# marius311/MuseInference.jl

Measured on AMD Instinct MI355X. Metric: MC sims/sec (MAP+score), higher is better.
Workload: dtype f64; 1 GPU; funnel_1e4: Neal's funnel family model=funnel, N=10000-dim z, 1-dim theta, nsims=512 per step (512 on this rank), cold start z0=0, atol=1e-2; element_split=1, parallelism=sims sharded over 1 GPU(s) (weak scaling), one all-gather of scores per step

## Files before the change

museinference.jl_amd/csrc/solver.hpp:

```cpp
#pragma once
#include <math.h>

#include "models.hpp"
#include "reduce.hpp"
#include "rng.hpp"

namespace muse {

template <int EPT>
struct Prefetch {
    int p;
    bool have_n1;
    bool have_n2;
    bool have_x;
    bool have_xg;
    bool g_pending;
};
#ifndef MUSE_NORMALS_AUX
#define MUSE_NORMALS_AUX 0
#endif
constexpr int kNormalsAux = MUSE_NORMALS_AUX;
typedef __attribute__((address_space(1))) const void* glds_src_t;
typedef __attribute__((address_space(3))) void* glds_dst_t;
template <int T, int EPT>
// ... 656 lines not shown
                dphi = trial_dphi;
                last_c = c;
                last_gmax = trial_gmax;
                last_phi = phi;
                f_calls += 1;
                return;
            }
        }
        double gm;
        if constexpr (!Place::kResident && !Model::kStencil) {
            if (z_zero) eval<true, false, false, true, kSpec>(c, phi, dphi, gm);
            else eval<true, false>(c, phi, dphi, gm);
        } else if constexpr (kSpec) {
            eval<true, false, false, false, true>(c, phi, dphi, gm);
        } else {
            eval<true, false>(c, phi, dphi, gm);
        }
        last_c = c;
        last_gmax = gm;
        last_phi = phi;
    }

    __device__ __forceinline__ static bool finite2(double p, double d) { return isfinite(p) && isfinite(d); }
    __device__ __forceinline__ static double eps_of(double b) {
        const double ab = fabs(b);
        return __longlong_as_double(__double_as_longlong(ab) + 1) - ab;
    }
    __device__ __forceinline__ static double nextup(double v) {
        if (v == 0.0) return 4.9406564584124654e-324;
        const long long b = __double_as_longlong(v);
        return __longlong_as_double(v > 0.0 ? b + 1 : b - 1);
    }
    __device__ __forceinline__ static bool wolfe(double c, double phi_c, double dphi_c, double phi_0, double dphi_0,
                                                 double phi_lim) {
        double delta = kHzDelta, sigma = kHzSigma, delta2 = 2.0 * kHzDelta - 1.0;
        if constexpr (Place::kResident) asm volatile("" : "+v"(delta), "+v"(sigma), "+v"(delta2));
        const bool w1 = (delta * dphi_0 >= (phi_c - phi_0) / c) && (dphi_c >= sigma * dphi_0);
        const bool w2 = (delta2 * dphi_0 >= dphi_c) && (dphi_c >= sigma * dphi_0) && (phi_c <= phi_lim);
        return w1 || w2;
    }
    __device__ __forceinline__ static double secant(const HzPoint& p, const HzPoint& q) {
        return (p.a * q.d - q.a * p.d) / (q.d - p.d);
    }

    __device__ __forceinline__ bool linesearch(double c0, double phi_0, double dphi_0, double& alpha) {
        enum { S_INIT, S_EXPAND, S_BIS, S_SEC1, S_SEC2, S_MID, S_FINAL };
        enum { CONT_BRACKET, CONT_UPD1, CONT_UPD2, CONT_UPD3 };
        alpha = 0.0;
        if (!finite2(phi_0, dphi_0)) return false;
        if (dphi_0 >= kEps * fabs(phi_0)) return false;
        if (dphi_0 >= 0.0 || c0 <= kEps) return true;
        const double phi_lim = phi_0 + kHzEpsilon * fabs(phi_0);
        const HzPoint P0{0.0, phi_0, dphi_0, 0};
        HzPoint A = P0, B = P0, C = P0, prev = P0, a0 = P0, b0 = P0;
        double alphamax = INFINITY, cold = 0.0, fail_alpha = 0.0, c = c0;
        int state = S_INIT, cont = CONT_BRACKET, iter = 1, iterfinite = 1, nid = 1;
        bool ok = true;
        for (;;) {
            double phi, dphi;
            if (iter_stamp < 3) stamp(stamp_p, 10 + 2 * iter_stamp);
            phidphi(c, phi, dphi);
            if (iter_stamp < 3) stamp(stamp_p, 11 + 2 * iter_stamp);
            iter_stamp += 1;
            const bool fin = finite2(phi, dphi);
            switch (state) {
                case S_INIT:
                    if (!fin) {
                        if (iterfinite < kHzIterFiniteMax) { iterfinite += 1; c *= kHzPsi3; continue; }
                        alpha = 0.0;
                        goto L_DONE;
                    }
                    C = HzPoint{c, phi, dphi, nid++};
                    goto L_BRACKET_TOP;
                case S_EXPAND:
                    if (!fin) {
                        if (c > nextup(cold) && iterfinite < kHzIterFiniteMax) {
                            alphamax = c;
                            iterfinite += 1;
                            c = (cold + c) / 2.0;
                            continue;
                        }
                        alpha = cold;
                        goto L_DONE;
                    }
                    C = HzPoint{c, phi, dphi, nid++};
                    iter += 1;
                    goto L_BRACKET_TOP;
                case S_BIS: {
                    if (!fin) goto L_FAIL;
                    const HzPoint D{c, phi, dphi, nid++};
                    if (D.d >= 0.0) { B = D; goto L_BISECT_RETURN; }
                    if (D.v <= phi_lim) A = D;
                    else B = D;
                    goto L_BISECT_TOP;
                }
                case S_SEC1:
                    if (!fin) goto L_FAIL;
                    C = HzPoint{c, phi, dphi, nid++};
                    if (wolfe(c, phi, dphi, phi_0, dphi_0, phi_lim)) { alpha = c; goto L_DONE; }
                    cont = CONT_UPD1;
                    goto L_UPDATE;
                case S_SEC2:
                    if (!fin) goto L_FAIL;
                    C = HzPoint{c, phi, dphi, nid++};
                    if (wolfe(c, phi, dphi, phi_0, dphi_0, phi_lim)) { alpha = c; goto L_DONE; }
                    cont = CONT_UPD2;
                    goto L_UPDATE;
                case S_MID:
                    if (!fin) goto L_FAIL;
                    C = HzPoint{c, phi, dphi, nid++};
                    cont = CONT_UPD3;
                    goto L_UPDATE;
                default:
                    return ok;
            }
        L_BRACKET_TOP:
            if (!(iter < kHzLinesearchMax)) { alpha = 0.0; goto L_FAIL_KEEP; }
            if (C.d >= 0.0) {
                A = prev;
                B = C;
                iter += 1;
                goto L_MAIN_TOP;
            } else if (C.v > phi_lim) {
                A = P0;
                B = C;
                cont = CONT_BRACKET;
                fail_alpha = 0.0;
                goto L_BISECT_ENTER;
            } else {
                cold = C.a;
                if (nextup(cold) >= alphamax) { alpha = cold; goto L_DONE; }
                prev = C;
                c = cold * kHzRho;
                if (c > alphamax) c = alphamax;
                iterfinite = 1;
                state = S_EXPAND;
                continue;
            }
        L_UPDATE:
            if (!(A.d < 0.0 && A.v <= phi_lim && B.d >= 0.0 && B.a > A.a)) goto L_FAIL;
            if (C.a < A.a || C.a > B.a) goto L_UPDATE_RETURN;
            if (C.d >= 0.0) { B = C; goto L_UPDATE_RETURN; }
            if (C.v <= phi_lim) { A = C; goto L_UPDATE_RETURN; }
            B = C;
        L_BISECT_ENTER:
            if (!(A.d < 0.0 && A.v <= phi_lim && B.d < 0.0 && B.v > phi_lim && B.a > A.a)) goto L_FAIL;
        L_BISECT_TOP:
            if (B.a - A.a > eps_of(B.a)) {
                c = (A.a + B.a) / 2.0;
                state = S_BIS;
                continue;
            }
        L_BISECT_RETURN:
            if (cont == CONT_BRACKET) { iter += 1; goto L_MAIN_TOP; }
        L_UPDATE_RETURN:
            if (cont == CONT_UPD1) {
                const bool updB = (B.id == C.id), updA = (A.id == C.id);
                double c2 = C.a;
                if (updB) c2 = secant(b0, B);
                else if (updA) c2 = secant(a0, A);
                if ((updA || updB) && A.a <= c2 && c2 <= B.a) {
                    c = c2;
                    state = S_SEC2;
                    continue;
                }
            }
            if (cont == CONT_UPD3) { iter += 1; goto L_MAIN_TOP; }
            if (!(B.a > A.a)) { alpha = A.a; goto L_FAIL_KEEP; }
            if (B.a - A.a < kHzGamma * (b0.a - a0.a)) {
                if (nextup(a0.v) >= b0.v && nextup(A.v) >= B.v) { alpha = A.a; goto L_DONE; }
                iter += 1;
                goto L_MAIN_TOP;
            }
            fail_alpha = A.a;
            c = (A.a + B.a) / 2.0;
            state = S_MID;
            continue;
        L_MAIN_TOP:
            if (!(iter < kHzLinesearchMax)) { alpha = A.a; goto L_FAIL_KEEP; }
            a0 = A;
            b0 = B;
            if (!(b0.a > a0.a)) { alpha = a0.a; goto L_FAIL_KEEP; }
            if (b0.a - a0.a <= eps_of(b0.a)) { alpha = a0.a; goto L_DONE; }
            fail_alpha = a0.a;
            if (!(a0.d < 0.0 && b0.d >= 0.0)) goto L_FAIL;
            c = secant(a0, b0);
            if (!isfinite(c)) goto L_FAIL;
            state = S_SEC1;
            continue;
        L_FAIL:
            alpha = fail_alpha;
        L_FAIL_KEEP:
            ok = false;
        L_DONE:
            if (!ok) return false;
            if (alpha == last_c) return true;
            c = alpha;
            state = S_FINAL;
        }
    }

    ProblemDesc d;
    double f, gmax;
    int iterations, hist_words, status;
    double* extra;

    __device__ __forceinline__ void run(int p, double* wg_scratch, double* lds_x, double* lds_g) {
        Prefetch<EPT> none;
        none.p = -1;
        none.g_pending = false;
        run(p, wg_scratch, lds_x, lds_g, none);
    }
    template <bool FD = true>
    __device__ __forceinline__ void run(int p, double* wg_scratch, double* lds_x, double* lds_g, Prefetch<EPT>& pf, int next_p = -1) {
        begin<false, FD>(p, wg_scratch, lds_x, lds_g, pf);
        if (d.normals_only) return;
        pfp = &pf;
        if constexpr (Place::kResident && Place::kXgLds) {
            if (next_p >= 0 && a.ncache_mode == 2 && !(a.debug & 4)) prefetch_issue<T>(a, tid, next_p, lds_x, lds_g, pf, false);
        }
        solve(p);
        finish(p);
        if constexpr (FD) {
            if (is_fid(p)) publish_fiducial();
        }
    }
    __device__ __forceinline__ bool is_fid(int p) const { return a.kind == BATCH_FD && a.fd_fold && p == 0; }
    __device__ __forceinline__ bool wait_fid(int p) const { return a.kind == BATCH_FD && a.fd_fold && p != 0; }
    __device__ __forceinline__ int info_row(int p) const {
        return (a.kind == BATCH_FD && a.fd_fold) ? (p == 0 ? a.nproblems - 1 : p - 1) : p;
    }
    __device__ __forceinline__ void publish_fiducial() {
        asm volatile("s_waitcnt vmcnt(0)" ::: "memory");
        __syncthreads();
        if (tid == 0) __hip_atomic_store(a.fid_flag, a.fid_tag, __ATOMIC_RELEASE, __HIP_MEMORY_SCOPE_AGENT);
    }
    __device__ __forceinline__ void wait_fiducial() {
        int* seen = reinterpret_cast<int*>(sh_rho + 40) + 2;
        if ((unsigned)__builtin_amdgcn_readfirstlane(seen[0]) == a.fid_tag) return;
        if ((__builtin_amdgcn_readfirstlane(tid) >> 6) == 0) {
            unsigned long long t0 = 0;
            unsigned spins = 0;
            while (__hip_atomic_load(a.fid_flag, __ATOMIC_RELAXED, __HIP_MEMORY_SCOPE_AGENT) != a.fid_tag) {
                __builtin_amdgcn_s_sleep(32);
                if ((++spins & 0x3fu) == 0) {
                    unsigned long long now;
                    asm volatile("s_memrealtime %0\n\ts_waitcnt lgkmcnt(0)" : "=s"(now)::"memory");
                    if (t0 == 0) t0 = now;
                    else if (now - t0 > 200000000ull) {
                        typedef __attribute__((address_space(1))) int gi32;
                        __hip_atomic_store((gi32*)a.error_flag, 1, __ATOMIC_RELAXED, __HIP_MEMORY_SCOPE_SYSTEM);
                        break;
                    }
                }
            }
        }
        __syncthreads();
        __builtin_amdgcn_fence(__ATOMIC_ACQUIRE, "agent");
        if (tid == 0) seen[0] = (int)a.fid_tag;
    }
#ifndef MUSE_KEEPZ_MAXB
#define MUSE_KEEPZ_MAXB 8
#endif
    static constexpr bool kKeepZ = Place::kResident && Place::kXgLds && !Model::kStencil && MAXB <= MUSE_KEEPZ_MAXB;
    __device__ __forceinline__ bool can_keep(int p) const {
        if constexpr (!kKeepZ) return false;
        const ProblemDesc dd = describe(a, p);
        return dd.z0_mode == Z0_WARM && !dd.normals_only && dd.tsample < 0 &&
               ((dd.x_mode == X_SAMPLE && dd.nslot >= 0 && a.ncache_mode == 2) || dd.x_mode == X_DATA);
    }
    __device__ __forceinline__ bool keeps_next(int p) const {
        if constexpr (!kKeepZ) return false;
        const ProblemDesc dd = describe(a, p);
        return !dd.normals_only && dd.tsample < 0 && dd.zslot >= 0 &&
               ((dd.x_mode == X_SAMPLE && dd.nslot >= 0 && a.ncache != nullptr && a.ncache_mode != 0) || dd.x_mode == X_DATA);
    }
    __device__ __forceinline__ void store_kept(int p) {
        if constexpr (kKeepZ) {
            const ProblemDesc dd = describe(a, p);
            if (dd.zslot < 0) return;
            const int64_t ld = a.ld;
            VH zout;
            zout.bind(a.zhat + dd.zslot * ld, ld);
            for_elems<T, EPT, U>(ld, tfirst, ps(), [&](int jj, int i) { zout.set(jj, i, z.get(jj, i)); });
        }
    }
    __device__ __forceinline__ void after_begin(int p, double* lds_x, double* lds_g, Prefetch<EPT>& pf, int next_p) {
        if (d.normals_only) return;
        pfp = &pf;
        if constexpr (Place::kResident && Place::kXgLds) {
            if (next_p >= 0 && a.ncache_mode == 2 && !(a.debug & 4)) prefetch_issue<T>(a, tid, next_p, lds_x, lds_g, pf, false);
        }
        solve(p);
        finish(p);
    }
    __device__ __forceinline__ void begin_kept(int p, double* wg_scratch, double* lds_x, double* lds_g, Prefetch<EPT>& pf) {
        if constexpr (kKeepZ) {
            d = describe(a, p);
            const bool pf_hit = pf.p == p;
            const int64_t N = a.N, ld = a.ld;
            init_done = false;
            z_zero = false;
            have_trial = false;
            stamp(p, 0);
            iv0 = a.cur.t.iv[0];
            sd0 = a.cur.t.sd[0];
            if constexpr (Model::kPair && MAXB == 2) {
                this->pc[0] = this->psd[0] = a.cur.t.sd[0];
                this->pc[1] = this->psd[1] = a.cur.t.sd[1];
                this->pc[2] = a.cur.t.sd[2];
                this->pc[3] = a.cur.t.sd[3];
            }
            if constexpr (MAXB > 1) {
                int tl = tid;
                asm volatile("" : "+v"(tl));
                if constexpr (Model::kPair) {
                    if (tl < MAXB) sh_sd[tl] = pair_table(a.cur.t)[4 * (tl >> 1) + (tl & 1)];
                } else {
                if (tl < MAXB) sh_sd[tl] = a.cur.t.sd[tl];
                }
                wg_barrier<true>();
            }
            hist = wg_scratch;
            x.bind(lds_x, ld);
            g.bind(lds_g, ld);
            if (d.x_mode == X_SAMPLE) {
                const rsrc_t n1r = make_rsrc(a.ncache + (int64_t)(2 * d.nslot) * ld, ld * 8);
                const rsrc_t n2r = make_rsrc(a.ncache + (int64_t)(2 * d.nslot + 1) * ld, ld * 8);
                int tl = tid;
                asm volatile("" : "+v"(tl));
                const bool n1_here = pf_hit && pf.have_n1, n2_here = pf_hit && pf.have_n2;
                if (n1_here && n2_here) {
                    asm volatile("s_waitcnt vmcnt(0)" ::: "memory");
#pragma unroll
                    for (int j = 0; j < EPT; ++j) {
                        const int i0 = 2 * (tl + j * T);
                        const double a0 = g.get(2 * j, i0), a1 = g.get(2 * j + 1, i0 + 1);
                        const double b0 = x.get(2 * j, i0), b1 = x.get(2 * j + 1, i0 + 1);
                        double zt0, xt0, zt1, xt1;
                        Model::sample(scoef(2 * j, i0), a0, b0, zt0, xt0, i0);
                        Model::sample(scoef(2 * j + 1, i0 + 1), a1, b1, zt1, xt1, i0 + 1);
                        const bool valid1 = i0 + 1 < (int)N;
                        if constexpr (Model::kPair) xt0 = i0 < (int)N ? xt0 : 0.0;
                        x.set(2 * j, i0, xt0);
                        x.set(2 * j + 1, i0 + 1, valid1 ? xt1 : 0.0);
                    }
                } else {
                    double c1[EPT][2], c2[EPT][2];
                    if (n1_here) asm volatile("s_waitcnt vmcnt(0)" ::: "memory");
                    if (!n2_here) {
#pragma unroll
                        for (int j = 0; j < EPT; ++j) load_f64x2<kNormalsAux>(n2r, 2 * (tl + j * T), c2[j][0], c2[j][1]);
                    }
                    if (!n1_here) {
#pragma unroll
                        for (int j = 0; j < EPT; ++j) load_f64x2<kNormalsAux>(n1r, 2 * (tl + j * T), c1[j][0], c1[j][1]);
                    }
                    if (n1_here) {
#pragma unroll
                        for (int j = 0; j < EPT; ++j) {
                            const int i0 = 2 * (tl + j * T);
                            c1[j][0] = g.get(2 * j, i0); c1[j][1] = g.get(2 * j + 1, i0 + 1);
                        }
                    }
                    if (n2_here) {
#pragma unroll
                        for (int j = 0; j < EPT; ++j) {
                            const int i0 = 2 * (tl + j * T);
                            c2[j][0] = x.get(2 * j, i0); c2[j][1] = x.get(2 * j + 1, i0 + 1);
                        }
                    }
#pragma unroll
                    for (int j = 0; j < EPT; ++j) {
                        const int i0 = 2 * (tl + j * T);
                        double zt0, xt0, zt1, xt1;
                        Model::sample(scoef(2 * j, i0), c1[j][0], c2[j][0], zt0, xt0, i0);
                        Model::sample(scoef(2 * j + 1, i0 + 1), c1[j][1], c2[j][1], zt1, xt1, i0 + 1);
                        const bool valid1 = i0 + 1 < (int)N;
                        if constexpr (Model::kPair) xt0 = i0 < (int)N ? xt0 : 0.0;
                        x.set(2 * j, i0, xt0);
                        x.set(2 * j + 1, i0 + 1, valid1 ? xt1 : 0.0);
                    }
                }
            } else {
                if (pf_hit && pf.have_x) {
                    asm volatile("s_waitcnt vmcnt(0)" ::: "memory");
                } else {
                    VH xs;
                    xs.bind(a.x_data, ld);
                    for_elems<T, EPT, U>(ld, tfirst, ps(), [&](int jj, int i) { x.set(jj, i, xs.get(jj, i)); }, x);
                }
            }
            s.clear();
            if (pf_hit) {
                pf.p = -1;
                pf.g_pending = false;
            }
            stamp(p, 9);
            wg_barrier<true>();
            stamp(p, 1);
        }
    }
    Prefetch<EPT>* pfp;
    __device__ __forceinline__ void drop_g_prefetch() {
        if constexpr (Place::kResident && Place::kXgLds) {
            if (pfp->g_pending) {
                asm volatile("s_waitcnt vmcnt(0)" ::: "memory");
                pfp->g_pending = false;
                pfp->p = -1;
            }
        }
    }

    __device__ __forceinline__ const SampleSd* tsample_base() const {
        if (a.tsample) return a.tsample;
        return reinterpret_cast<const SampleSd*>(reinterpret_cast<const char*>((const void*)__builtin_amdgcn_kernarg_segment_ptr()) +
                                                 offsetof(BatchArgs, maps));
    }
    template <bool KEEP_ZTRUE>
    __device__ __forceinline__ void begin(int p, double* wg_scratch, double* lds_x, double* lds_g) {
        Prefetch<EPT> none;
        none.p = -1;
        none.g_pending = false;
        pfp = nullptr;
        begin<KEEP_ZTRUE>(p, wg_scratch, lds_x, lds_g, none);
    }
    template <bool KEEP_ZTRUE, bool FD = true>
    __device__ __forceinline__ void begin(int p, double* wg_scratch, double* lds_x, double* lds_g, Prefetch<EPT>& pf) {
        d = describe(a, p);
        const bool pf_hit = Place::kResident && Place::kXgLds && pf.p == p;
        const int64_t N = a.N, ld = a.ld;
        init_done = false;
        z_zero = false;
        have_trial = false;
        stamp(p, 0);
        iv0 = a.cur.t.iv[0];
        sd0 = d.tsample >= 0 ? tsample_base()[d.tsample].sd[0] : a.cur.t.sd[0];
        if constexpr (Model::kPair && MAXB == 2) {
            this->pc[0] = a.cur.t.sd[0];
            this->pc[1] = a.cur.t.sd[1];
            this->pc[2] = a.cur.t.sd[2];
            this->pc[3] = a.cur.t.sd[3];
            this->psd[0] = sd0;
            this->psd[1] = d.tsample >= 0 ? tsample_base()[d.tsample].sd[1] : a.cur.t.sd[1];
        }
        if constexpr (kBig) {
            const BigTheta* bt = reinterpret_cast<const BigTheta*>(
                reinterpret_cast<const char*>((const void*)__builtin_amdgcn_kernarg_segment_ptr()) + offsetof(BatchArgs, big));
            big_iv = bt->iv;
            big_sd = d.tsample >= 0 ? reinterpret_cast<const double*>(a.tsample) + (int64_t)d.tsample * kBigTheta : bt->sd;
            big_rcpN = 1.0 / (double)a.N;
        } else if constexpr (MAXB > 1) {
            int tl = tid;
            asm volatile("" : "+v"(tl));
            if constexpr (Model::kPair) {
                if (tl < MAXB) sh_sd[tl] = d.tsample >= 0 ? tsample_base()[d.tsample].sd[tl] : pair_table(a.cur.t)[4 * (tl >> 1) + (tl & 1)];
            } else {
            if (tl < MAXB) sh_sd[tl] = d.tsample >= 0 ? tsample_base()[d.tsample].sd[tl] : a.cur.t.sd[tl];
            }
            wg_barrier<!Model::kStencil>();
        }
        const double* zmem = nullptr;
        if constexpr (Place::kResident) {
            hist = wg_scratch;
            if constexpr (Place::kXgLds) {
                x.bind(lds_x, ld);
                g.bind(lds_g, ld);
            }
        } else {
            double* xbuf = wg_scratch;
            double* sbuf = wg_scratch + 2 * ld;
            if constexpr (kBg) {
                if (bufsel) {
                    xbuf = wg_scratch + (int64_t)(4 + 2 * kM + 1) * ld;
                    sbuf = xbuf + ld;
                }
            }
            x.bind(xbuf, ld);
            g.bind(wg_scratch + ld, ld);
            if constexpr (Place::kLdsS) s.bind(wg_scratch + 2 * ld, ld, lds_x, tfirst, pstride, tid, (int)N);
            else s.bind(sbuf, ld);
            zmem = d.zslot >= 0 ? a.zhat + d.zslot * ld : wg_scratch + 3 * ld;
            z.bind(zmem, ld);
            hist = wg_scratch + 4 * ld;
            extra = hist + (int64_t)2 * kM * ld;
        }
        const double* z0ptr = a.zhat + d.z0slot * ld;
        VH z0src;
        z0src.bind(z0ptr, ld);
        const bool z_in_place = (!Place::kResident) && (d.z0_mode == Z0_WARM || d.z0_mode == Z0_COPY) && (z0ptr == zmem);

        if (d.x_mode == X_SAMPLE) {
            const uint64_t sim = (uint64_t)d.sim;
            if constexpr (Place::kResident && Place::kXgLds) {
                const int nmode = d.nslot >= 0 ? a.ncache_mode : 0;
                rsrc_t n1r = make_rsrc(a.ncache, 0), n2r = n1r;
                if (nmode != 0) {
                    n1r = make_rsrc(a.ncache + (int64_t)(2 * d.nslot) * ld, ld * 8);
                    n2r = make_rsrc(a.ncache + (int64_t)(2 * d.nslot + 1) * ld, ld * 8);
                }
                const bool z_warm = d.z0_mode != Z0_ZERO && d.z0_mode != Z0_TRUE;
                bool z_loaded = false;
                double zw[EPT][2];
                if (nmode == 2) {
                    double c1[EPT][2], c2[EPT][2];
                    int tl = tid;
                    asm volatile("" : "+v"(tl));
                    const bool n1_here = pf_hit && pf.have_n1, n2_here = pf_hit && pf.have_n2;
                    if (n1_here) asm volatile("s_waitcnt vmcnt(0)" ::: "memory");
                    const bool fold_wait = FD && wait_fid(p);
                    if (z_warm && !fold_wait) {
#pragma unroll
                        for (int j = 0; j < EPT; ++j) load_f64x2(z0src.rsrc, 2 * (tl + j * T), zw[j][0], zw[j][1]);
                        z_loaded = true;
                    }
                    if (!n2_here) {
#pragma unroll
                        for (int j = 0; j < EPT; ++j) load_f64x2<kNormalsAux>(n2r, 2 * (tl + j * T), c2[j][0], c2[j][1]);
                    }
                    if (!n1_here) {
#pragma unroll
                        for (int j = 0; j < EPT; ++j) load_f64x2<kNormalsAux>(n1r, 2 * (tl + j * T), c1[j][0], c1[j][1]);
                    }
                    if (n1_here) {
#pragma unroll
                        for (int j = 0; j < EPT; ++j) {
                            const int i0 = 2 * (tl + j * T);
                            c1[j][0] = g.get(2 * j, i0); c1[j][1] = g.get(2 * j + 1, i0 + 1);
                        }
                    }
                    if (n2_here) {
#pragma unroll
                        for (int j = 0; j < EPT; ++j) {
                            const int i0 = 2 * (tl + j * T);
                            c2[j][0] = x.get(2 * j, i0); c2[j][1] = x.get(2 * j + 1, i0 + 1);
                        }
                    }
                    const bool stage_ztrue = d.z0_mode == Z0_TRUE;
#pragma unroll
                    for (int j = 0; j < EPT; ++j) {
                        const int i0 = 2 * (tl + j * T);
                        double zt0, xt0, zt1, xt1;
                        Model::sample(scoef(2 * j, i0), c1[j][0], c2[j][0], zt0, xt0, i0);
                        Model::sample(scoef(2 * j + 1, i0 + 1), c1[j][1], c2[j][1], zt1, xt1, i0 + 1);
                        const bool valid1 = i0 + 1 < (int)N;
                        if constexpr (Model::kPair) {
                            const bool valid0 = i0 < (int)N;
                            xt0 = valid0 ? xt0 : 0.0;
                            zt0 = valid0 ? zt0 : 0.0;
                        }
                        x.set(2 * j, i0, xt0);
                        x.set(2 * j + 1, i0 + 1, valid1 ? xt1 : 0.0);
                        if (stage_ztrue) {
                            g.set(2 * j, i0, zt0);
                            g.set(2 * j + 1, i0 + 1, valid1 ? zt1 : 0.0);
                        }
                    }
                    if (z_warm && fold_wait) {
                        wait_fiducial();
#pragma unroll
                        for (int j = 0; j < EPT; ++j) load_f64x2(z0src.rsrc, 2 * (tl + j * T), zw[j][0], zw[j][1]);
                        z_loaded = true;
                    }
                } else {
                    auto sd_of = [&](int jj) {
                        if constexpr (MAXB == 1) return sd0;
                        else {
                            const unsigned w = jj >= 10 ? pk[1] : pk[0];
                            const int sh = 3 * (jj >= 10 ? jj - 10 : jj);
                            if constexpr (Model::kPair) return scoef_of_block((int)((w >> sh) & 7u));
                            else return sh_sd[(w >> sh) & 7u];
                        }
                    };
                    auto draw = [&](auto npairs, int i0, int j) {
                        constexpr int P = decltype(npairs)::value;
                        uint64_t idx[2 * P];
                        NormalPair np[2 * P];
#pragma unroll
                        for (int q = 0; q < P; ++q) {
                            idx[2 * q] = (uint64_t)(i0 + 2 * T * q);
                            idx[2 * q + 1] = (uint64_t)(i0 + 2 * T * q + 1);
                        }
                        normal_pairs<2 * P>(a.seed, sim, idx, np);
#pragma unroll
                        for (int q = 0; q < P; ++q) {
                            const int j0 = i0 + 2 * T * q;
                            if (nmode == 1) {
                                store_f64x2(n1r, j0, np[2 * q].n1, np[2 * q + 1].n1);
                                store_f64x2(n2r, j0, np[2 * q].n2, np[2 * q + 1].n2);
                            }
                            double zt0, xt0, zt1, xt1;
                            Model::sample(sd_of(2 * (j + q)), np[2 * q].n1, np[2 * q].n2, zt0, xt0, j0);
                            Model::sample(sd_of(2 * (j + q) + 1), np[2 * q + 1].n1, np[2 * q + 1].n2, zt1, xt1, j0 + 1);
                            const bool valid1 = j0 + 1 < (int)N;
                            x.p[j0] = xt0;
                            g.p[j0] = zt0;
                            x.p[j0 + 1] = valid1 ? xt1 : 0.0;
                            g.p[j0 + 1] = valid1 ? zt1 : 0.0;
                        }
                    };
                    int j = 0;
                    int tl = tid;
                    asm volatile("" : "+v"(tl));
#pragma unroll 1
                    for (int i0 = 2 * tl; i0 < (int)N; i0 += 2 * T * kSamplerPairs, j += kSamplerPairs) {
                        if constexpr (kSamplerPairs == 2) {
                            if (i0 + 2 * T < (int)N) draw(std::integral_constant<int, 2>{}, i0, j);
                            else draw(std::integral_constant<int, 1>{}, i0, j);
                        } else {
                            draw(std::integral_constant<int, 1>{}, i0, j);
                        }
                    }
                }
                z.clear();
                s.clear();
                if (z_loaded) {
#pragma unroll
                    for (int j = 0; j < EPT; ++j) {
                        z.set(2 * j, 0, zw[j][0]);
                        z.set(2 * j + 1, 0, zw[j][1]);
                    }
                } else {
                    for_elems<T, EPT, U>(ld, tfirst, ps(), [&](int jj, int i) {
                        if (d.z0_mode == Z0_ZERO) z.set(jj, i, 0.0);
                        else if (d.z0_mode == Z0_TRUE) z.set(jj, i, g.get(jj, i));
                        else z.set(jj, i, z0src.get(jj, i));
                    });
                }
            } else {
                x.clear(); g.clear(); z.clear(); s.clear();
                VH ztrue;
                if constexpr (KEEP_ZTRUE) ztrue.bind(extra, ld);
                constexpr int US = Place::kResident ? U : 1;
                const bool z_from_sample = d.z0_mode == Z0_ZERO || d.z0_mode == Z0_TRUE;
                if constexpr (kBg && !KEEP_ZTRUE) {
                    if (d.z0_mode == Z0_ZERO && !d.normals_only && d.tsample < 0) {
                        if (gen.p != p) {
                            gen.p = p;
                            gen.trip = 0;
                            gen.sim = sim;
#pragma unroll
                            for (int k = 0; k < 4; ++k) gen.sum[k] = 0.0;
                            gen.mx[0] = gen.mx[1] = 0.0;
                        }
                        gen.active = false;
                        const int ntrips = gen_trips();
#pragma unroll 1
                        for (; gen.trip < ntrips; ++gen.trip) {
                            const int i0 = 2 * (tfirst + gen.trip * pstride);
                            double xo[2], so[2];
                            gen_pair(i0, xo, so);
                            store_f64x2(x.rsrc, i0, xo[0], xo[1]);
                            store_f64x2(s.rsrc, i0, so[0], so[1]);
                        }
                        double sum[4] = {gen.sum[0], gen.sum[1], gen.sum[2], gen.sum[3]}, mx[2] = {gen.mx[0], gen.mx[1]};
                        reduce<4, 2>(sum, mx);
                        init_f = 0.5 * (sum[0] + a.cur.f_const);
                        init_dphi = sum[1];
                        init_gmax = nan_if(sum[0] != sum[0] || sum[1] != sum[1], mx[0]);
                        trial_c = 1.0;
                        trial_phi = 0.5 * (sum[2] + a.cur.f_const);
                        trial_dphi = sum[3];
                        trial_gmax = nan_if(sum[2] != sum[2] || sum[3] != sum[3], mx[1]);
                        init_done = true;
                        z_zero = true;
                    }
                }
                if constexpr (!Model::kStencil) {
                    if (!init_done && z_from_sample && !d.normals_only) {
                        const bool ztrue_start = d.z0_mode == Z0_TRUE;
                        double sum[4] = {0.0, 0.0, 0.0, 0.0}, mx[2] = {0.0, 0.0};
                        constexpr int kGenU = Place::kResident ? 1 : kStreamGenU;
                        NormalPair npv[2 * kGenU];
                        for_elems_pre<T, EPT, kGenU>(ld, tfirst, ps(), [&](auto ucount, int i0, int pstr) {
                            constexpr int UU = decltype(ucount)::value;
                            uint64_t idx[2 * UU];
                            NormalPair got[2 * UU];
#pragma unroll
                            for (int u = 0; u < UU; ++u) {
                                idx[2 * u] = (uint64_t)(i0 + 2 * u * pstr);
                                idx[2 * u + 1] = (uint64_t)(i0 + 2 * u * pstr + 1);
                            }
                            normal_pairs<2 * UU>(a.seed, sim, idx, got);
#pragma unroll
                            for (int q = 0; q < 2 * UU; ++q) npv[q] = got[q];
                        }, [&](int jj, int i) {
                            const bool valid = i < N;
                            const NormalPair np = npv[jj % (2 * kGenU)];
                            double zt, xt;
                            Model::sample(scoef(jj, i), np.n1, np.n2, zt, xt, i);
                            zt = valid ? zt : 0.0;
                            xt = valid ? xt : 0.0;
                            if constexpr (KEEP_ZTRUE) ztrue.set(jj, i, keep_value(valid, zt, sdk(jj, i), np, i));
                            x.set(jj, i, xt);
                            const double z0v = ztrue_start ? zt : 0.0;
                            if (Place::kResident || ztrue_start) z.set(jj, i, z0v);
                            const auto ivi = gcoef(jj, i);
                            const double gi = Model::grad(ivi, xt, z0v, sum[0], i);
                            const double sd = -gi;
                            s.set(jj, i, sd);
                            sum[1] = fma(gi, sd, sum[1]);
                            mx[0] = absmax(mx[0], gi);
                            const double zt1 = fma(1.0, sd, z0v);
                            const double gt = Model::grad(ivi, xt, zt1, sum[2], i);
                            sum[3] = fma(gt, sd, sum[3]);
                            mx[1] = absmax(mx[1], gt);
                        }, when(KEEP_ZTRUE, ztrue), x, s, when(Place::kResident || ztrue_start, z));
                        reduce<4, 2>(sum, mx);
                        init_f = 0.5 * (sum[0] + a.cur.f_const);
                        init_dphi = sum[1];
                        init_gmax = nan_if(sum[0] != sum[0] || sum[1] != sum[1], mx[0]);
                        trial_c = 1.0;
                        trial_phi = 0.5 * (sum[2] + a.cur.f_const);
                        trial_dphi = sum[3];
                        trial_gmax = nan_if(sum[2] != sum[2] || sum[3] != sum[3], mx[1]);
                        init_done = true;
                        z_zero = !ztrue_start && !Place::kResident;
                    }
                }
                if (!init_done)
                for_elems<T, EPT, US>(ld, tfirst, ps(), [&](int jj, int i) {
                    const bool valid = i < N;
                    const NormalPair np = normal_pair(a.seed, sim, (uint64_t)i);
                    double zt, xt;
                    if constexpr (Model::kStencil) {
                        zt = sdk(jj, i) * np.n1;
                        xt = np.n2;
                        g.set(jj, i, valid ? zt : 0.0);
                    } else {
                        Model::sample(scoef(jj, i), np.n1, np.n2, zt, xt, i);
                    }
                    zt = valid ? zt : 0.0;
                    xt = valid ? xt : 0.0;
                    if constexpr (KEEP_ZTRUE) ztrue.set(jj, i, keep_value(valid, zt, sdk(jj, i), np, i));
                    x.set(jj, i, xt);
                    if (d.z0_mode == Z0_ZERO) z.set(jj, i, 0.0);
                    else if (d.z0_mode == Z0_TRUE) z.set(jj, i, zt);
                    else if constexpr (Place::kResident) z.set(jj, i, z0src.get(jj, i));
                }, when(Model::kStencil, g), when(KEEP_ZTRUE, ztrue), x, when(z_from_sample, z));
                if constexpr (!Place::kResident) {
                    if (!init_done && !z_from_sample && !z_in_place)
                        for_elems<T, EPT, U>(ld, tfirst, ps(), [&](int jj, int i) { z.set(jj, i, z0src.get(jj, i)); }, z);
                }
            }
            if constexpr (Model::kStencil) {
                pass_barrier();
                const NoiseVec<Model, 1> sn;
                for_elems<T, EPT, U>(ld, tfirst, ps(), [&](int jj, int i) {
                    const bool valid = i < N;
                    const int ic = valid ? i : 0;
                    const int im = ic == 0 ? (int)N - 1 : ic - 1, ip = ic == (int)N - 1 ? 0 : ic + 1;
                    const double zl = g.get1(im), zr = g.get1(ip);
                    const double az = stencil_apply<Model>(zl, g.get1(ic), zr);
                    if constexpr (noise_model<Model>()) {
                        const double si = sn.get(jj, i);
                        const double xv = fma(si, x.get(jj, i), az);
                        x.set(jj, i, valid && si != 0.0 ? xv : 0.0);
                    } else {
                        const double xv = az + x.get(jj, i);
                        x.set(jj, i, valid ? xv : 0.0);
                    }
                }, x);
            }
        } else {
            VH xs;
            xs.bind(d.x_mode == X_DATA ? a.x_data : a.x_given, ld);
            x.clear(); g.clear(); z.clear(); s.clear();
            const bool z_zero = d.z0_mode == Z0_ZERO || d.z0_mode == Z0_TRUE;
            bool done = false;
            if constexpr (Place::kResident && Place::kXgLds) {
                if (pf_hit && pf.have_x && d.x_mode == X_DATA && !z_zero) {
                    asm volatile("s_waitcnt vmcnt(0)" ::: "memory");
                    for_elems<T, EPT, U>(ld, tfirst, ps(), [&](int jj, int i) { z.set(jj, i, z0src.get(jj, i)); });
                    done = true;
                } else if (pf_hit && pf.have_xg && d.x_mode == X_DATA && !z_zero) {
                    asm volatile("s_waitcnt vmcnt(0)" ::: "memory");
                    for_elems<T, EPT, U>(ld, tfirst, ps(), [&](int jj, int i) {
                        x.set(jj, i, g.get(jj, i));
                        z.set(jj, i, z0src.get(jj, i));
                    });
                    done = true;
                }
            }
            if (!done)
            for_elems<T, EPT, U>(ld, tfirst, ps(), [&](int jj, int i) {
                x.set(jj, i, xs.get(jj, i));
                if (z_zero) z.set(jj, i, 0.0);
                else if (!z_in_place) z.set(jj, i, z0src.get(jj, i));
            }, x, when(z_zero || !z_in_place, z));
        }
        if (pf_hit) {
            if constexpr (Place::kResident && Place::kXgLds) {
                if (pf.g_pending) asm volatile("s_waitcnt vmcnt(0)" ::: "memory");
            }
            pf.p = -1;
            pf.g_pending = false;
        }
        stamp(p, 9);
        if constexpr (Model::kStencil) pass_barrier();
        else wg_barrier<true>();
        if constexpr (kBg && !KEEP_ZTRUE) {
            gen.active = false;
            const bool same_map = a.nmaps <= 1 || next_p / a.n_per_map == p / a.n_per_map;
            if (next_p >= 0 && d.tsample < 0 && same_map) {
                const ProblemDesc dn = describe(a, next_p);
                if (dn.x_mode == X_SAMPLE && dn.z0_mode == Z0_ZERO && !dn.normals_only && dn.tsample < 0) {
                    gen.p = next_p;
                    gen.trip = 0;
                    gen.sim = (uint64_t)dn.sim;
#pragma unroll
                    for (int k = 0; k < 4; ++k) gen.sum[k] = 0.0;
                    gen.mx[0] = gen.mx[1] = 0.0;
                    gen.active = true;
                    double* xb = bufsel ? wg_scratch : wg_scratch + (int64_t)(4 + 2 * kM + 1) * ld;
                    double* sb = bufsel ? wg_scratch + 2 * ld : xb + ld;
                    bg_xr = make_rsrc(xb, ld * 8);
                    bg_sr = make_rsrc(sb, ld * 8);
                }
            }
        }

        stamp(p, 1);
    }

    static constexpr bool kPrefetchTwoLoop = !Place::kResident && Place::kCluster && Model::kStencil;
    template <class F>
    __device__ __forceinline__ void pass_ab(VH& A, VH& B, F&& f) {
        int t = tfirst;
        asm volatile("" : "+v"(t));
        const int n = (int)a.ld, pstr = pstride;
#pragma unroll 1
        for (int i0 = 2 * t; i0 < n; i0 += 2 * U * pstr) {
#pragma unroll
            for (int u = 0; u < U; ++u) {
                const int i = i0 + 2 * u * pstr;
                f(2 * u, i);
                f(2 * u + 1, i + 1);
            }
            s.template flush<U>(i0, pstr);
            A.unload();
            B.unload();
        }
    }
    __device__ __forceinline__ double twoloop_prefetched(int upper, int lower, double dot0) {
        if constexpr (kPrefetchTwoLoop) {
            double dot = dot0;
            int t0 = tfirst;
            asm volatile("" : "+v"(t0));
            auto fetch = [&](VH& v) { v.template preload<U>(2 * t0, pstride); };
            VH A = hdg((upper - 1) % kM), B = A;
            if (upper > lower) B = hdx((upper - 2) % kM);
            for (int index = upper; index >= lower; --index) {
                const int slot = (index - 1) % kM;
                const double al = sh_rho[slot] * dot;
                if ((tid & 63) == 0) sh_alpha[slot] = al;
                double sum[1] = {0.0}, mx[1] = {0.0};
                if (index > lower) {
                    pass_ab(A, B, [&](int jj, int i) {
                        const double qi = fma(-al, A.get(jj, i), s.get(jj, i));
                        s.set(jj, i, qi);
                        sum[0] = fma(B.get(jj, i), qi, sum[0]);
                    });
                } else {
                    const double gam = sh_gam[(upper - 1) % kM];
                    pass_ab(A, B, [&](int jj, int i) {
                        const double dgi = A.get(jj, i);
                        const double si = gam * fma(-al, dgi, s.get(jj, i));
                        s.set(jj, i, si);
                        sum[0] = fma(dgi, si, sum[0]);
                    });
                }
                if (index > lower) {
                    A = hdg((index - 2) % kM);
                    fetch(A);
                    if (index - 1 > lower) {
                        B = hdx((index - 3) % kM);
                        fetch(B);
                    }
                } else {
                    A = hdx((lower - 1) % kM);
                    fetch(A);
                    if (lower < upper) {
                        B = hdg(lower % kM);
                        fetch(B);
                    } else {
                        fetch(g);
                    }
                }
                reduce<1, 0>(sum, mx);
                dot = sum[0];
            }
            for (int index = lower; index <= upper; ++index) {
                const int slot = (index - 1) % kM;
                const double beta = sh_rho[slot] * dot;
                const double coef = sh_alpha[slot] - beta;
                double sum[1] = {0.0}, mx[1] = {0.0};
                if (index < upper) {
                    pass_ab(A, B, [&](int jj, int i) {
                        const double si = fma(A.get(jj, i), coef, s.get(jj, i));
                        s.set(jj, i, si);
                        sum[0] = fma(B.get(jj, i), si, sum[0]);
                    });
                    A = hdx(index % kM);
                    fetch(A);
                    if (index + 1 < upper) {
                        B = hdg((index + 1) % kM);
                        fetch(B);
                    } else {
                        fetch(g);
                    }
                } else {
                    pass_ab(A, g, [&](int jj, int i) {
                        const double si = -fma(A.get(jj, i), coef, s.get(jj, i));
                        s.set(jj, i, si);
                        sum[0] = fma(g.get(jj, i), si, sum[0]);
                    });
                }
                reduce<1, 0>(sum, mx);
                dot = sum[0];
            }
            return dot;
        } else {
            (void)upper; (void)lower;
            return dot0;
        }
    }

    __device__ __forceinline__ void solve(int p) {
        const int64_t ld = a.ld;
        const int N = (int)a.N;
        f_calls = 0;
// ... 735 lines not shown
```

Baseline: 11.04 million sims/s.

## Fuse initial gradient and first trial-step evaluation into the cold-start sampling loop

For cold starts with z0=0 on non-stencil models, the sampling loop now computes the initial gradient, the steepest-descent direction, and a unit-step trial gradient inline while the data is being drawn. It reduces these into the initial and trial objective and gradient-max values, so the solver can skip the separate first init and line-search pass. The staged ztrue values are written to g only when z0 starts from the true sample, which saves a store otherwise. This adds register pressure and a fixed unit trial step to the sampling loop, and relies on the solver honouring the precomputed init and trial state.

```diff
diff --git a/museinference.jl_amd/csrc/solver.hpp b/museinference.jl_amd/csrc/solver.hpp
--- a/museinference.jl_amd/csrc/solver.hpp
+++ b/museinference.jl_amd/csrc/solver.hpp
@@ -982,6 +982,8 @@
             init_done = false;
             z_zero = false;
             have_trial = false;
+            init_f = init_dphi = init_gmax = 0.0;
+            trial_phi = trial_dphi = trial_gmax = 0.0;
             stamp(p, 0);
             iv0 = a.cur.t.iv[0];
             sd0 = a.cur.t.sd[0];
@@ -1113,6 +1115,10 @@
         init_done = false;
         z_zero = false;
         have_trial = false;
+        if constexpr (Place::kResident && Place::kXgLds) {
+            init_f = init_dphi = init_gmax = 0.0;
+            trial_phi = trial_dphi = trial_gmax = 0.0;
+        }
         stamp(p, 0);
         iv0 = a.cur.t.iv[0];
         sd0 = d.tsample >= 0 ? tsample_base()[d.tsample].sd[0] : a.cur.t.sd[0];
@@ -1252,7 +1258,28 @@
                             else return sh_sd[(w >> sh) & 7u];
                         }
                     };
-                    auto draw = [&](auto npairs, int i0, int j) {
+                    const bool fuse_init = __builtin_amdgcn_readfirstlane(
+                        (int)(!Model::kStencil && d.z0_mode == Z0_ZERO && !d.normals_only && !(a.debug & 1024))) != 0;
+                    const bool stage_ztrue = d.z0_mode == Z0_TRUE;
+                    double isum[4] = {0.0, 0.0, 0.0, 0.0}, imx[2] = {0.0, 0.0};
+                    auto gcoef_of = [&](int jj, int i) {
+                        if constexpr (MAXB == 1 || (Model::kPair && MAXB == 2)) return gcoef(jj, i);
+                        else {
+                            const unsigned w = jj >= 10 ? pk[1] : pk[0];
+                            const int sh = 3 * (jj >= 10 ? jj - 10 : jj);
+                            const int b = (int)((w >> sh) & 7u);
+                            if constexpr (Model::kPair) {
+                                PairGp c;
+                                c.p = pair_table(a.cur.t) + 4 * b;
+                                c.valid = i < (int)N;
+                                return c;
+                            } else {
+                                return a.cur.t.iv[b];
+                            }
+                        }
+                    };
+                    auto draw = [&](auto fused, auto npairs, int i0, int j) {
+                        constexpr bool FUSED = decltype(fused)::value;
                         constexpr int P = decltype(npairs)::value;
                         uint64_t idx[2 * P];
                         NormalPair np[2 * P];
@@ -1273,23 +1300,61 @@
                             Model::sample(sd_of(2 * (j + q)), np[2 * q].n1, np[2 * q].n2, zt0, xt0, j0);
                             Model::sample(sd_of(2 * (j + q) + 1), np[2 * q + 1].n1, np[2 * q + 1].n2, zt1, xt1, j0 + 1);
                             const bool valid1 = j0 + 1 < (int)N;
+                            xt1 = valid1 ? xt1 : 0.0;
                             x.p[j0] = xt0;
-                            g.p[j0] = zt0;
-                            x.p[j0 + 1] = valid1 ? xt1 : 0.0;
-                            g.p[j0 + 1] = valid1 ? zt1 : 0.0;
+                            x.p[j0 + 1] = xt1;
+                            if constexpr (FUSED) {
+                                const double xe[2] = {xt0, xt1};
+                                double se[2];
+#pragma unroll
+                                for (int v = 0; v < 2; ++v) {
+                                    const double zi = 0.0, xi = xe[v];
+                                    const auto ivi = gcoef_of(2 * (j + q) + v, j0 + v);
+                                    const double gi = Model::grad(ivi, xi, zi, isum[0], j0 + v);
+                                    const double sd = -gi;
+                                    se[v] = sd;
+                                    isum[1] = fma(gi, sd, isum[1]);
+                                    imx[0] = absmax(imx[0], gi);
+                                    const double zt = fma(1.0, sd, zi);
+                                    const double gt = Model::grad(ivi, xi, zt, isum[2], j0 + v);
+                                    isum[3] = fma(gt, sd, isum[3]);
+                                    imx[1] = absmax(imx[1], gt);
+                                }
+                                g.p[j0] = se[0];
+                                g.p[j0 + 1] = se[1];
+                            } else if (stage_ztrue) {
+                                g.p[j0] = zt0;
+                                g.p[j0 + 1] = valid1 ? zt1 : 0.0;
+                            }
                         }
                     };
-                    int j = 0;
-                    int tl = tid;
-                    asm volatile("" : "+v"(tl));
+                    auto draw_all = [&](auto fused) {
+                        int j = 0;
+                        int tl = tid;
+                        asm volatile("" : "+v"(tl));
 #pragma unroll 1
-                    for (int i0 = 2 * tl; i0 < (int)N; i0 += 2 * T * kSamplerPairs, j += kSamplerPairs) {
-                        if constexpr (kSamplerPairs == 2) {
-                            if (i0 + 2 * T < (int)N) draw(std::integral_constant<int, 2>{}, i0, j);
-                            else draw(std::integral_constant<int, 1>{}, i0, j);
-                        } else {
-                            draw(std::integral_constant<int, 1>{}, i0, j);
+                        for (int i0 = 2 * tl; i0 < (int)N; i0 += 2 * T * kSamplerPairs, j += kSamplerPairs) {
+                            if constexpr (kSamplerPairs == 2) {
+                                if (i0 + 2 * T < (int)N) draw(fused, std::integral_constant<int, 2>{}, i0, j);
+                                else draw(fused, std::integral_constant<int, 1>{}, i0, j);
+                            } else {
+                                draw(fused, std::integral_constant<int, 1>{}, i0, j);
+                            }
                         }
+                    };
+                    if (fuse_init) {
+                        draw_all(std::true_type{});
+                        reduce<4, 2>(isum, imx);
+                        init_f = uniform(0.5 * (isum[0] + a.cur.f_const));
+                        init_dphi = isum[1];
+                        init_gmax = uniform(nan_if(isum[0] != isum[0] || isum[1] != isum[1], imx[0]));
+                        trial_c = 1.0;
+                        trial_phi = uniform(0.5 * (isum[2] + a.cur.f_const));
+                        trial_dphi = isum[3];
+                        trial_gmax = uniform(nan_if(isum[2] != isum[2] || isum[3] != isum[3], imx[1]));
+                        init_done = true;
+                    } else {
+                        draw_all(std::false_type{});
                     }
                 }
                 z.clear();
@@ -1307,6 +1372,7 @@
                         else z.set(jj, i, z0src.get(jj, i));
                     });
                 }
+                if (init_done) for_elems<T, EPT, U>(ld, tfirst, ps(), [&](int jj, int i) { s.set(jj, i, g.get(jj, i)); });
             } else {
                 x.clear(); g.clear(); z.clear(); s.clear();
                 VH ztrue;
```

New measurement: 11.21 million sims/s (median of 4 runs). +1.5%, better.
